# zhengchen1999/DOVE

Hardware: AMD Instinct MI355X
Metric: SR frames/s (33x720x1280 4x one-step, whole job) (higher is better)
Workload: dtype bf16; 1 GPU; synthetic 33x720x1280 HR clip (LR 180x320, 4x), one-step t=399, CogVideoX1.5-5B VAE + 42-layer DiT random-init, 1 clip per GPU (BASELINE configs[1]); weight_sums=True, vae_streams=2, variant=headline (bf16)

## Files before the change

### dove_amd/csrc/elementwise.hip

```cpp
#include "common.h"
#include "../../include/dove_hip.h"

__device__ __forceinline__ float load_any(const void* p, long long i, int dt) {
  return dt == DOVE_F32 ? ((const float*)p)[i] : bf2f(((const bf16_t*)p)[i]);
}
__device__ __forceinline__ void store_any(void* p, long long i, int dt, float v) {
  if (dt == DOVE_F32) ((float*)p)[i] = v;
  else ((bf16_t*)p)[i] = f2bf(v);
}

__global__ void cl_from_ncthw_kernel(const void* __restrict__ x, int dt, int C, long long npix, int Cp,
                                     float scale, float shift, bf16_t* __restrict__ y) {
  const long long p = (long long)blockIdx.x * blockDim.x + threadIdx.x;
  if (p >= npix) return;
  bf16_t* yr = y + p * Cp;
  for (int c0 = 0; c0 < Cp; c0 += 8) {
    float f[8];
#pragma unroll
    for (int e = 0; e < 8; ++e) {
      const int c = c0 + e;
      f[e] = c < C ? load_any(x, (long long)c * npix + p, dt) * scale + shift : 0.f;
    }
    *(uint4*)(yr + c0) = pack8(f);
  }
}

extern "C" int dove_cl_from_ncthw(const void* x, int dtype, int C, long long npix, int Cp, float scale, float shift,
                                   void* y, void* stream) {
  DOVE_CHECK_ARG(x && y, "cl_from_ncthw: null pointer");
  DOVE_CHECK_ARG(dtype == DOVE_F32 || dtype == DOVE_BF16, "cl_from_ncthw: bad dtype %d", dtype);
  DOVE_CHECK_ARG(Cp % 8 == 0 && Cp >= C && C > 0 && npix > 0, "cl_from_ncthw: need Cp %% 8 == 0, Cp >= C");
  hipLaunchKernelGGL(cl_from_ncthw_kernel, dim3((unsigned)((npix + 255) / 256)), dim3(256), 0, (hipStream_t)stream, x,
                     dtype, C, npix, Cp, scale, shift, (bf16_t*)y);
  DOVE_CHECK_LAUNCH("dove_cl_from_ncthw");
  return DOVE_OK;
}

__global__ void cl_im2col3x3_kernel(const void* __restrict__ x, int dt, int C, int T, int H, int W, int Cp, float scale, float shift,
                                    bf16_t* __restrict__ y) {
  const long long npix = (long long)T * H * W;
  const long long p = (long long)blockIdx.x * blockDim.x + threadIdx.x;
  if (p >= npix) return;
  const int w = (int)(p % W), h = (int)((p / W) % H);
  bf16_t* yr = y + p * Cp;
  for (int c0 = 0; c0 < Cp; c0 += 8) {
    float f[8];
#pragma unroll
    for (int e = 0; e < 8; ++e) {
      const int k = c0 + e, tap = k / C, c = k - tap * C;
      const int dy = tap / 3 - 1, dx = tap % 3 - 1;
      const bool in = tap < 9 && h + dy >= 0 && h + dy < H && w + dx >= 0 && w + dx < W;
      f[e] = in ? load_any(x, (long long)c * npix + p + (long long)dy * W + dx, dt) * scale + shift : 0.f;
    }
    *(uint4*)(yr + c0) = pack8(f);
  }
}
extern "C" int dove_cl_im2col3x3_from_ncthw(const void* x, int dtype, int C, int T, int H, int W, int Cp, float scale, float shift, void* y,
                                            void* stream) {
  DOVE_CHECK_ARG(x && y, "cl_im2col3x3: null pointer");
  DOVE_CHECK_ARG(dtype == DOVE_F32 || dtype == DOVE_BF16, "cl_im2col3x3: bad dtype %d", dtype);
  DOVE_CHECK_ARG(C > 0 && Cp % 8 == 0 && Cp >= 9 * C && T > 0 && H > 0 && W > 0, "cl_im2col3x3: need Cp %% 8 == 0 and Cp >= 9 C");
  const long long npix = (long long)T * H * W;
  hipLaunchKernelGGL(cl_im2col3x3_kernel, dim3((unsigned)((npix + 255) / 256)), dim3(256), 0, (hipStream_t)stream, x, dtype, C, T, H, W, Cp,
                     scale, shift, (bf16_t*)y);
  DOVE_CHECK_LAUNCH("dove_cl_im2col3x3_from_ncthw");
  return DOVE_OK;
}

__global__ void ncthw_from_cl_kernel(const bf16_t* __restrict__ x, long long ld, int C, long long npix, float scale,
                                     float shift, float lo, float hi, void* __restrict__ y, int dt) {
  const long long p = (long long)blockIdx.x * blockDim.x + threadIdx.x;
  if (p >= npix) return;
  const bf16_t* xr = x + p * ld;
  for (int c0 = 0; c0 < C; c0 += 4) {
    const uint2 v = *(const uint2*)(xr + c0);
    const float f[4] = {__uint_as_float(v.x << 16), __uint_as_float(v.x & 0xffff0000u), __uint_as_float(v.y << 16),
                        __uint_as_float(v.y & 0xffff0000u)};
#pragma unroll
    for (int e = 0; e < 4; ++e)
      if (c0 + e < C) store_any(y, (long long)(c0 + e) * npix + p, dt, fminf(fmaxf(f[e] * scale + shift, lo), hi));
  }
}

extern "C" int dove_ncthw_from_cl(const void* x, long long ld, int C, long long npix, float scale, float shift,
                                   float lo, float hi, void* y, int dtype, void* stream) {
  DOVE_CHECK_ARG(x && y, "ncthw_from_cl: null pointer");
  DOVE_CHECK_ARG(dtype == DOVE_F32 || dtype == DOVE_BF16, "ncthw_from_cl: bad dtype %d", dtype);
  DOVE_CHECK_ARG(ld % 4 == 0 && ld >= ((C + 3) / 4) * 4 && C > 0 && npix > 0, "ncthw_from_cl: ld must be a multiple of 4 covering C");
  hipLaunchKernelGGL(ncthw_from_cl_kernel, dim3((unsigned)((npix + 255) / 256)), dim3(256), 0, (hipStream_t)stream,
                     (const bf16_t*)x, ld, C, npix, scale, shift, lo, hi, y, dtype);
  DOVE_CHECK_LAUNCH("dove_ncthw_from_cl");
  return DOVE_OK;
}

__global__ __launch_bounds__(256) void conv_out_gather_kernel(const float* __restrict__ p, int ldp, int T, int H, int W, int C,
                                                              const float* __restrict__ bias, float scale, float shift, float lo, float hi,
                                                              void* __restrict__ y, int dt, int ldy) {
  extern __shared__ __attribute__((aligned(16))) float tile[];
  constexpr int TH = 8, TW = 64, RW = TW + 2, NREC = (TH + 2) * RW;
  const int lrec = ldp + 1, f4n = ldp >> 2;
  const int x0 = blockIdx.x * TW, y0 = blockIdx.y * TH, t = blockIdx.z;
  for (int i = threadIdx.x; i < NREC * f4n; i += 256) {
    const int rec = i / f4n, f4 = i - rec * f4n;
    const int ry = rec / RW, rx = rec - ry * RW;
    const int iy = y0 + ry - 1, ix = x0 + rx - 1;
    f32x4 v = {0.f, 0.f, 0.f, 0.f};
    if (iy >= 0 && iy < H && ix >= 0 && ix < W) v = *(const f32x4*)(p + (((long long)t * H + iy) * W + ix) * ldp + f4 * 4);
    float* d = tile + rec * lrec + f4 * 4;
    d[0] = v[0]; d[1] = v[1]; d[2] = v[2]; d[3] = v[3];
  }
  __syncthreads();
  const int lx = threadIdx.x & 63;
  const long long npix = (long long)T * H * W;
#pragma unroll
  for (int h2 = 0; h2 < 2; ++h2) {
    const int rr = (threadIdx.x >> 6) + 4 * h2;
    const int oy = y0 + rr, ox = x0 + lx;
    if (oy >= H || ox >= W) continue;
    float acc[4] = {0.f, 0.f, 0.f, 0.f};
#pragma unroll
    for (int dy = 0; dy < 3; ++dy)
#pragma unroll
      for (int dx = 0; dx < 3; ++dx) {
        const float* q = tile + ((rr + dy) * RW + lx + dx) * lrec + (dy * 3 + dx) * C;
        for (int c = 0; c < C; ++c) acc[c] += q[c];
      }
    const long long pix = ((long long)t * H + oy) * W + ox;
    if (ldy > 0) {
      bf16_t* yp = (bf16_t*)y + pix * ldy;
      for (int c = 0; c < ldy; ++c) yp[c] = c < C ? f2bf(acc[c] + (bias ? bias[c] : 0.f)) : (bf16_t)0;
      continue;
    }
    for (int c = 0; c < C; ++c) {
      const float v = bf2f(f2bf(acc[c] + (bias ? bias[c] : 0.f)));
      store_any(y, (long long)c * npix + pix, dt, fminf(fmaxf(v * scale + shift, lo), hi));
    }
  }
}
static int conv_out_gather_launch(const float* p, long long ldp, int T, int H, int W, int C, const float* bias, float scale, float shift,
                                  float lo, float hi, void* y, int dtype, int ldy, void* stream) {
  DOVE_CHECK_ARG(p && y, "conv_out_gather: null pointer");
  DOVE_CHECK_ARG(C >= 1 && C <= 4 && ldp >= 9 * C && ldp <= 36 && ldp % 4 == 0 && T > 0 && H > 0 && W > 0,
                 "conv_out_gather: need 1 <= C <= 4 and 9 C <= ldp <= 36, ldp %% 4 == 0");
  const int lds = 10 * 66 * ((int)ldp + 1) * 4;
  static PerDeviceOnce attr;
  if (auto once_ = attr.guard()) { (void)hipFuncSetAttribute((const void*)conv_out_gather_kernel, hipFuncAttributeMaxDynamicSharedMemorySize, 10 * 66 * 37 * 4); }
  dim3 grid((unsigned)((W + 63) / 64), (unsigned)((H + 7) / 8), (unsigned)T);
  hipLaunchKernelGGL(conv_out_gather_kernel, grid, dim3(256), lds, (hipStream_t)stream, p, (int)ldp, T, H, W, C, bias, scale, shift, lo, hi, y, dtype, ldy);
  DOVE_CHECK_LAUNCH("dove_conv_out_gather");
  return DOVE_OK;
}
extern "C" int dove_conv_out_gather(const float* p, long long ldp, int T, int H, int W, int C, const float* bias, float scale, float shift,
                                    float lo, float hi, void* y, int dtype, void* stream) {
  DOVE_CHECK_ARG(dtype == DOVE_F32 || dtype == DOVE_BF16, "conv_out_gather: bad dtype %d", dtype);
  return conv_out_gather_launch(p, ldp, T, H, W, C, bias, scale, shift, lo, hi, y, dtype, 0, stream);
}
extern "C" int dove_conv_out_gather_cl(const float* p, long long ldp, int T, int H, int W, int C, const float* bias, void* y, int ldy, void* stream) {
  DOVE_CHECK_ARG(ldy >= C && ldy <= 32 && ldy % 4 == 0, "conv_out_gather_cl: need C <= ldy <= 32, ldy %% 4 == 0 (got %d)", ldy);
  DOVE_CHECK_ARG(T <= 65535, "conv_out_gather_cl: more than 65535 frames (%d) in one call", T);
  return conv_out_gather_launch(p, ldp, T, H, W, C, bias, 1.0f, 0.0f, 0.0f, 0.0f, y, DOVE_BF16, ldy, stream);
}

__host__ __device__ inline int odd_to(int T) { return (T & 1) ? 1 + (T - 1) / 2 : T / 2; }
__global__ void avgpool_time_kernel(const bf16_t* __restrict__ x, int T, long long frame8, bf16_t* __restrict__ y) {
  const long long i = (long long)blockIdx.x * blockDim.x + threadIdx.x;
  if (i >= frame8) return;
  const int To = odd_to(T);
  const int inst = blockIdx.y / To, to = blockIdx.y - inst * To;
  const int odd = T & 1;
  const uint4* xs = (const uint4*)x + (long long)inst * T * frame8;
  uint4* ys = (uint4*)y + (long long)inst * To * frame8;
  if (odd && to == 0) {
    ys[i] = xs[i];
    return;
  }
  const int t0 = odd ? 1 + 2 * (to - 1) : 2 * to;
  float a[8], b[8];
  unpack8(xs[(long long)t0 * frame8 + i], a);
  unpack8(xs[(long long)(t0 + 1) * frame8 + i], b);
#pragma unroll
  for (int e = 0; e < 8; ++e) a[e] = 0.5f * (a[e] + b[e]);
  ys[(long long)to * frame8 + i] = pack8(a);
}

extern "C" int dove_avgpool_time_nb_bf16(const void* x, int nb, int T, long long frame_elems, void* y, void* stream) {
  DOVE_CHECK_ARG(x && y, "avgpool_time: null pointer");
  DOVE_CHECK_ARG(T >= 2 && frame_elems % 8 == 0 && frame_elems > 0, "avgpool_time: need T >= 2 and frame_elems %% 8 == 0");
  const int To = odd_to(T);
  DOVE_CHECK_ARG(nb >= 1 && (long long)nb * To <= 65535, "avgpool_time: bad instance count %d", nb);
  const long long f8 = frame_elems / 8;
  hipLaunchKernelGGL(avgpool_time_kernel, dim3((unsigned)((f8 + 255) / 256), nb * To), dim3(256), 0, (hipStream_t)stream,
                     (const bf16_t*)x, T, f8, (bf16_t*)y);
  DOVE_CHECK_LAUNCH("dove_avgpool_time_bf16");
  return DOVE_OK;
}
extern "C" int dove_avgpool_time_bf16(const void* x, int T, long long frame_elems, void* y, void* stream) {
  return dove_avgpool_time_nb_bf16(x, 1, T, frame_elems, y, stream);
}

__global__ void posterior_kernel(const bf16_t* __restrict__ mom, long long ld, int L, long long npix,
                                 const void* __restrict__ noise, int ndt, void* __restrict__ out, int odt) {
  const long long p = (long long)blockIdx.x * blockDim.x + threadIdx.x;
  if (p >= npix) return;
  for (int c = 0; c < L; ++c) {
    const float mean = bf2f(mom[p * ld + c]);
    float lv = bf2f(mom[p * ld + L + c]);
    lv = fminf(fmaxf(lv, -30.f), 20.f);
    const float eps = load_any(noise, (long long)c * npix + p, ndt);
    store_any(out, (long long)c * npix + p, odt, mean + __expf(0.5f * lv) * eps);
  }
}

extern "C" int dove_posterior_sample(const void* moments, long long ld, int latent_channels, long long npix,
                                      const void* noise, int noise_dtype, void* out, int out_dtype, void* stream) {
  DOVE_CHECK_ARG(moments && noise && out, "posterior_sample: null pointer");
  DOVE_CHECK_ARG(ld >= 2 * latent_channels && npix > 0, "posterior_sample: bad ld");
  hipLaunchKernelGGL(posterior_kernel, dim3((unsigned)((npix + 255) / 256)), dim3(256), 0, (hipStream_t)stream,
                     (const bf16_t*)moments, ld, latent_channels, npix, noise, noise_dtype, out, out_dtype);
  DOVE_CHECK_LAUNCH("dove_posterior_sample");
  return DOVE_OK;
}

__global__ void axpby_kernel(const void* x, const void* y, void* out, int dt, long long n, float a, float b) {
  const long long i = (long long)blockIdx.x * blockDim.x + threadIdx.x;
  if (i >= n) return;
  store_any(out, i, dt, a * load_any(x, i, dt) + b * load_any(y, i, dt));
}

extern "C" int dove_axpby(const void* x, const void* y, void* out, int dtype, long long n, float a, float b,
                           void* stream) {
  DOVE_CHECK_ARG(x && y && out && n > 0, "axpby: null pointer / empty");
  DOVE_CHECK_ARG(dtype == DOVE_F32 || dtype == DOVE_BF16, "axpby: bad dtype %d", dtype);
  hipLaunchKernelGGL(axpby_kernel, dim3((unsigned)((n + 255) / 256)), dim3(256), 0, (hipStream_t)stream, x, y, out,
                     dtype, n, a, b);
  DOVE_CHECK_LAUNCH("dove_axpby");
  return DOVE_OK;
}

__global__ void patchify_kernel(const void* __restrict__ x, int dt, int T, int C, int H, int W, int pt, int p,
                                bf16_t* __restrict__ tok, long long ld, int dir, void* __restrict__ y) {
  const int gh = H / p, gw = W / p;
  const int F = C * pt * p * p;
  const long long total = (long long)(T / pt) * gh * gw * F;
  const long long i = (long long)blockIdx.x * blockDim.x + threadIdx.x;
  if (i >= total) return;
  const int f = (int)(i % F);
  const long long n = i / F;
  const int pw = f % p, ph = (f / p) % p, tt = (f / (p * p)) % pt, c = f / (p * p * pt);
  const int iw = (int)(n % gw), ih = (int)((n / gw) % gh), it = (int)(n / ((long long)gw * gh));
  const long long src = (((long long)(it * pt + tt) * C + c) * H + ih * p + ph) * W + iw * p + pw;
  if (dir == 0) tok[n * ld + f] = f2bf(load_any(x, src, dt));
  else store_any(y, src, dt, bf2f(tok[n * ld + f]));
}

extern "C" int dove_patchify(const void* x, int dtype, int T, int C, int H, int W, int pt, int p, void* tokens,
                              long long ld, void* stream) {
  DOVE_CHECK_ARG(x && tokens, "patchify: null pointer");
  DOVE_CHECK_ARG(T % pt == 0 && H % p == 0 && W % p == 0 && ld >= (long long)C * pt * p * p, "patchify: shape not divisible by patch");
  const long long total = (long long)(T / pt) * (H / p) * (W / p) * C * pt * p * p;
  hipLaunchKernelGGL(patchify_kernel, dim3((unsigned)((total + 255) / 256)), dim3(256), 0, (hipStream_t)stream, x,
                     dtype, T, C, H, W, pt, p, (bf16_t*)tokens, ld, 0, nullptr);
  DOVE_CHECK_LAUNCH("dove_patchify");
  return DOVE_OK;
}

extern "C" int dove_unpatchify(const void* tokens, long long ld, int T, int C, int H, int W, int pt, int p, void* y,
                                int dtype, void* stream) {
  DOVE_CHECK_ARG(y && tokens, "unpatchify: null pointer");
  DOVE_CHECK_ARG(T % pt == 0 && H % p == 0 && W % p == 0 && ld >= (long long)C * pt * p * p, "unpatchify: shape not divisible by patch");
  const long long total = (long long)(T / pt) * (H / p) * (W / p) * C * pt * p * p;
  hipLaunchKernelGGL(patchify_kernel, dim3((unsigned)((total + 255) / 256)), dim3(256), 0, (hipStream_t)stream,
                     nullptr, dtype, T, C, H, W, pt, p, (bf16_t*)const_cast<void*>(tokens), ld, 1, y);
  DOVE_CHECK_LAUNCH("dove_unpatchify");
  return DOVE_OK;
}

__global__ __launch_bounds__(256) void gemv_kernel(const bf16_t* __restrict__ W, const float* __restrict__ b,
                                                   const float* __restrict__ x, int in_f, int out_f, int act,
                                                   float* __restrict__ y) {
  const int lane = threadIdx.x & 63;
  const int j = blockIdx.x * 4 + (threadIdx.x >> 6);
  if (j >= out_f) return;
  const bf16_t* wr = W + (long long)j * in_f;
  float acc = 0.f;
  for (int k0 = lane * 8; k0 < in_f; k0 += 512) {
    float w[8];
    unpack8(*(const uint4*)(wr + k0), w);
#pragma unroll
    for (int e = 0; e < 8; ++e) {
      float xv = x[k0 + e];
      if (act == 1) xv = silu_f(xv);
      acc += w[e] * xv;
    }
  }
  acc = wave_sum(acc);
  if (lane == 0) y[j] = acc + (b ? b[j] : 0.f);
}

extern "C" int dove_gemv_bf16(const void* W, const float* bias, const float* x, int in_features, int out_features,
                               int act_in, float* y, void* stream) {
  DOVE_CHECK_ARG(W && x && y, "gemv: null pointer");
// ... 169 lines not shown
```

### dove_amd/csrc/norm.hip

```cpp
#include "common.h"
#include "../../include/dove_hip.h"

__global__ __launch_bounds__(256) void gn_partial_kernel(const bf16_t* __restrict__ xall, long long npix, int C,
                                                         int cpp_log, float* __restrict__ partial_all) {
  const bf16_t* __restrict__ x = xall + (long long)blockIdx.y * npix * C;
  float* __restrict__ partial = partial_all + (long long)blockIdx.y * gridDim.x * 64;
  __shared__ float red[256 * 17];
  __shared__ float chan[2 * 2048];
  const int tid = threadIdx.x;
  const int cpp = 1 << cpp_log;
  const int q = tid & (cpp - 1), sub = tid >> cpp_log;
  const int nsub = 256 >> cpp_log;
  float s[8], ss[8];
#pragma unroll
  for (int e = 0; e < 8; ++e) { s[e] = 0.f; ss[e] = 0.f; }
  for (long long p = (long long)blockIdx.x * nsub + sub; p < npix; p += (long long)gridDim.x * nsub) {
    const uint4 v = *(const uint4*)(x + p * C + q * 8);
    float f[8];
    unpack8(v, f);
#pragma unroll
    for (int e = 0; e < 8; ++e) { s[e] += f[e]; ss[e] += f[e] * f[e]; }
  }
  float* r = red + (q * nsub + sub) * 17;
#pragma unroll
// ... 130 lines not shown
  while ((1 << cpp_log) < C / 8) ++cpp_log;
  const int nsub = 256 >> cpp_log;
  long long bpf = (frame_pix + (long long)nsub * 32 - 1) / ((long long)nsub * 32);
  if (bpf > 256) bpf = 256;
  if (bpf * frames > ws_blocks) {
    dove_set_error("%s: %lld frames x %lld blocks per frame exceed the %d scratch rows", who, frames, bpf, ws_blocks);
    return 0;
  }
  hipLaunchKernelGGL(gn_partial_kernel, dim3((unsigned)bpf, (unsigned)frames), dim3(256), 0, s, (const bf16_t*)x, frame_pix, C, cpp_log,
                     (float*)partial_ws);
  return (int)(bpf * frames);
}

extern "C" int dove_groupnorm_stats_bf16(const void* x, long long npix, long long frame_pix, int C, float eps, void* partial_ws,
                                          int ws_blocks, float* stats, void* stream) {
  DOVE_CHECK_ARG(x && partial_ws && stats, "groupnorm_stats: null pointer");
  hipStream_t s = (hipStream_t)stream;
  const int rows = gn_partial_launch(x, npix, frame_pix, C, partial_ws, ws_blocks, s, "groupnorm_stats");
  if (!rows) return DOVE_EINVAL;
  DOVE_CHECK_LAUNCH("dove_groupnorm_stats_bf16(partial)");
  hipLaunchKernelGGL(gn_finalize_kernel<float>, dim3(1), dim3(256), 0, s, (const float*)partial_ws, rows,
                     (double)npix * (double)(C / 32), eps, stats);
  DOVE_CHECK_LAUNCH("dove_groupnorm_stats_bf16(finalize)");
  return DOVE_OK;
}

extern "C" int dove_groupnorm_stats_nb_bf16(const void* x, int nb, long long npix, long long frame_pix, int C, float eps, void* partial_ws,
                                             int ws_blocks, float* stats, void* stream) {
  DOVE_CHECK_ARG(x && partial_ws && stats && nb >= 1, "groupnorm_stats: null pointer");
  hipStream_t s = (hipStream_t)stream;
  const int rows = gn_partial_launch(x, npix * nb, frame_pix > 0 ? frame_pix : npix, C, partial_ws, ws_blocks, s, "groupnorm_stats");
  if (!rows) return DOVE_EINVAL;
  DOVE_CHECK_LAUNCH("dove_groupnorm_stats_bf16(partial)");
  DOVE_CHECK_ARG(rows % nb == 0, "groupnorm_stats: %d partial rows do not split over %d instances", rows, nb);
  hipLaunchKernelGGL(gn_finalize_kernel<float>, dim3(nb), dim3(256), 0, s, (const float*)partial_ws, rows / nb,
                     (double)npix * (double)(C / 32), eps, stats);
  DOVE_CHECK_LAUNCH("dove_groupnorm_stats_bf16(finalize)");
  return DOVE_OK;
}

extern "C" int dove_groupnorm_sums_bf16(const void* x, long long npix, long long frame_pix, int C, void* partial_ws, int ws_blocks,
                                        double* sums, void* stream) {
  DOVE_CHECK_ARG(x && partial_ws && sums, "groupnorm_sums: null pointer");
  hipStream_t s = (hipStream_t)stream;
  const int rows = gn_partial_launch(x, npix, frame_pix, C, partial_ws, ws_blocks, s, "groupnorm_sums");
  if (!rows) return DOVE_EINVAL;
  DOVE_CHECK_LAUNCH("dove_groupnorm_sums_bf16(partial)");
  hipLaunchKernelGGL(gn_sums_kernel<float>, dim3(1), dim3(256), 0, s, (const float*)partial_ws, rows, sums);
  DOVE_CHECK_LAUNCH("dove_groupnorm_sums_bf16(sums)");
  return DOVE_OK;
}

struct GnApplyArgs {
  const bf16_t* x; bf16_t* y; const float* stats; const float* gamma; const float* beta;
  const bf16_t* yb;
  int T, H, W, C, cpp_log;
  int hz, wz, sshift;
  int tmap[32];
  int act;
  int Tz;
};

__global__ __launch_bounds__(256) void gn_apply_kernel(const GnApplyArgs a) {
  const int tid = threadIdx.x;
  const int cpp = 1 << a.cpp_log;
  const int q = tid & (cpp - 1), sub = tid >> a.cpp_log;
  const int nsub = 256 >> a.cpp_log;
  const int cpg = a.C / 32;
  const int t = blockIdx.y;
  const int b = t / a.T;
  const float* __restrict__ stats = a.stats + b * 64;
  float sc[8], sh[8];
#pragma unroll
  for (int e = 0; e < 8; ++e) {
    const int ch = q * 8 + e, g = ch / cpg;
    const float mean = stats[g * 2], rstd = stats[g * 2 + 1];
    sc[e] = rstd * a.gamma[ch];
    sh[e] = a.beta[ch] - mean * sc[e];
  }
  const int tz = b * a.Tz + a.tmap[t - b * a.T];
  for (int h = blockIdx.x; h < a.H; h += gridDim.x) {
    const long long rowbase = ((long long)t * a.H + h) * a.W;
    const long long zrow = ((long long)tz * a.hz + (h >> a.sshift)) * a.wz;
    for (int w0 = sub; w0 < a.W; w0 += 4 * nsub) {
      uint4 xv[4], yv[4], bv[4];
#pragma unroll
      for (int u = 0; u < 4; ++u) {
        const int w = w0 + u * nsub;
        if (w < a.W) {
          xv[u] = *(const uint4*)(a.x + (rowbase + w) * a.C + q * 8);
          if (a.yb) {
            const bf16_t* yb = a.yb + (zrow + (w >> a.sshift)) * (2 * a.C) + q * 8;
            yv[u] = *(const uint4*)yb;
            bv[u] = *(const uint4*)(yb + a.C);
          }
        }
      }
#pragma unroll
      for (int u = 0; u < 4; ++u) {
        const int w = w0 + u * nsub;
        if (w < a.W) {
          float f[8];
          unpack8(xv[u], f);
#pragma unroll
          for (int e = 0; e < 8; ++e) f[e] = f[e] * sc[e] + sh[e];
          if (a.yb) {
            float fy[8], fb[8];
            unpack8(yv[u], fy);
            unpack8(bv[u], fb);
#pragma unroll
            for (int e = 0; e < 8; ++e) f[e] = f[e] * fy[e] + fb[e];
          }
          if (a.act) {
#pragma unroll
            for (int e = 0; e < 8; ++e) f[e] = silu_f(f[e]);
          }
          *(uint4*)(a.y + (rowbase + w) * a.C + q * 8) = pack8(f);
        }
      }
    }
  }
}

extern "C" int dove_groupnorm_apply_nb_bf16(const void* x, void* y, int nb, int T, int H, int W, int C, const float* stats,
                                             const float* gamma, const float* beta, int silu, const void* yb, int Tz, int hz,
                                             int wz, int sshift, const int* tmap, void* stream) {
  DOVE_CHECK_ARG(x && y && stats && gamma && beta, "groupnorm_apply: null pointer");
  DOVE_CHECK_ARG(nb >= 1 && (long long)nb * T <= 65535, "groupnorm_apply: bad instance count %d", nb);
  DOVE_CHECK_ARG(C >= 32 && C <= 2048 && (C & (C - 1)) == 0, "groupnorm_apply: C (%d) must be a power of two in [32,2048]", C);
  DOVE_CHECK_ARG(T > 0 && T <= 32 && H > 0 && W > 0, "groupnorm_apply: need 0 < T <= 32 frames per batch (got %d), H, W > 0", T);
  GnApplyArgs a;
  a.x = (const bf16_t*)x; a.y = (bf16_t*)y; a.stats = stats; a.gamma = gamma; a.beta = beta; a.yb = (const bf16_t*)yb;
  a.T = T; a.H = H; a.W = W; a.C = C; a.act = silu;
  int cpp_log = 0;
  while ((1 << cpp_log) < C / 8) ++cpp_log;
  a.cpp_log = cpp_log;
  a.hz = hz; a.wz = wz; a.sshift = sshift; a.Tz = Tz;
  for (int i = 0; i < 32; ++i) a.tmap[i] = 0;
  if (yb) {
    DOVE_CHECK_ARG(tmap, "groupnorm_apply: spatial norm needs a frame map");
    DOVE_CHECK_ARG(sshift >= 0 && sshift <= 8 && (hz << sshift) >= H && (wz << sshift) >= W, "groupnorm_apply: latent grid too small");
    for (int i = 0; i < T; ++i) a.tmap[i] = tmap[i];
  }
  hipLaunchKernelGGL(gn_apply_kernel, dim3(H < 4096 ? H : 4096, nb * T), dim3(256), 0, (hipStream_t)stream, a);
  DOVE_CHECK_LAUNCH("dove_groupnorm_apply_bf16");
  return DOVE_OK;
}
extern "C" int dove_groupnorm_apply_bf16(const void* x, void* y, int T, int H, int W, int C, const float* stats,
                                          const float* gamma, const float* beta, int silu, const void* yb, int hz,
                                          int wz, int sshift, const int* tmap, void* stream) {
  return dove_groupnorm_apply_nb_bf16(x, y, 1, T, H, W, C, stats, gamma, beta, silu, yb, 0, hz, wz, sshift, tmap, stream);
}

template <int NIT>
__global__ __launch_bounds__(256) void ln_mod_kernel(const bf16_t* __restrict__ x, bf16_t* __restrict__ y,
                                                     long long rows, int D, float eps,
                                                     const float* __restrict__ gamma, const float* __restrict__ beta,
                                                     const float* __restrict__ mod, long long split) {
  extern __shared__ __attribute__((aligned(16))) float lnp[];
  float* A = lnp;
  float* Bv = lnp + 2 * D;
  for (int c = threadIdx.x; c < D; c += 256) {
    const float g = gamma[c], b = beta[c];
#pragma unroll
    for (int cls = 0; cls < 2; ++cls) {
      float sc = 0.f, sh = 0.f;
      if (mod) { sh = mod[(long long)cls * 2 * D + c]; sc = mod[(long long)cls * 2 * D + D + c]; }
      A[cls * D + c] = g * (1.0f + sc);
      Bv[cls * D + c] = b * (1.0f + sc) + sh;
    }
  }
  __syncthreads();
  const int lane = threadIdx.x & 63, wave = threadIdx.x >> 6;
  for (int r = 0; r < 8; ++r) {
    const long long row = (long long)blockIdx.x * 32 + wave * 8 + r;
    if (row >= rows) break;
    const bf16_t* xr = x + row * D;
    float f[NIT][8];
    float s = 0.f;
#pragma unroll
    for (int i = 0; i < NIT; ++i) {
      const int c0 = (i * 64 + lane) * 8;
      if (c0 < D) {
        unpack8(*(const uint4*)(xr + c0), f[i]);
#pragma unroll
        for (int e = 0; e < 8; ++e) s += f[i][e];
      } else {
#pragma unroll
        for (int e = 0; e < 8; ++e) f[i][e] = 0.f;
      }
    }
    const float mean = wave_sum(s) / (float)D;
    float v = 0.f;
#pragma unroll
    for (int i = 0; i < NIT; ++i) {
      const int c0 = (i * 64 + lane) * 8;
      if (c0 < D) {
#pragma unroll
        for (int e = 0; e < 8; ++e) { const float d = f[i][e] - mean; v += d * d; }
      }
    }
    const float rstd = rsqrtf(wave_sum(v) / (float)D + eps);
    const int cls = row < split ? 0 : 1;
    bf16_t* yr = y + row * D;
#pragma unroll
    for (int i = 0; i < NIT; ++i) {
      const int c0 = (i * 64 + lane) * 8;
      if (c0 < D) {
        const f32x4 a0 = *(const f32x4*)(A + cls * D + c0), a1 = *(const f32x4*)(A + cls * D + c0 + 4);
        const f32x4 b0 = *(const f32x4*)(Bv + cls * D + c0), b1 = *(const f32x4*)(Bv + cls * D + c0 + 4);
        float o[8];
#pragma unroll
        for (int e = 0; e < 4; ++e) {
          o[e] = (f[i][e] - mean) * rstd * a0[e] + b0[e];
          o[4 + e] = (f[i][4 + e] - mean) * rstd * a1[e] + b1[e];
        }
        *(uint4*)(yr + c0) = pack8(o);
      }
    }
  }
}

extern "C" int dove_layernorm_modulate_bf16(const void* x, void* y, long long rows, int D, float eps,
                                             const float* gamma, const float* beta, const float* mod,
                                             long long split, void* stream) {
  DOVE_CHECK_ARG(x && y && gamma && beta, "layernorm_modulate: null pointer");
  DOVE_CHECK_ARG(D % 8 == 0 && D > 0 && D <= 4096, "layernorm_modulate: D (%d) must be a multiple of 8, <= 4096", D);
  DOVE_CHECK_ARG(rows > 0, "layernorm_modulate: empty input");
  const int nit = (D + 511) / 512;
  const unsigned grid = (unsigned)((rows + 31) / 32);
  const size_t lds = (size_t)4 * D * sizeof(float);
  hipStream_t s = (hipStream_t)stream;
#define LN_LAUNCH(N)                                                                                          \
  hipLaunchKernelGGL((ln_mod_kernel<N>), dim3(grid), dim3(256), lds, s, (const bf16_t*)x, (bf16_t*)y, rows, D, eps, \
                     gamma, beta, mod, split)
  switch (nit) {
    case 1: LN_LAUNCH(1); break;
    case 2: LN_LAUNCH(2); break;
    case 3: LN_LAUNCH(3); break;
    case 4: LN_LAUNCH(4); break;
    case 5: LN_LAUNCH(5); break;
    case 6: LN_LAUNCH(6); break;
    case 7: LN_LAUNCH(7); break;
    default: LN_LAUNCH(8); break;
  }
#undef LN_LAUNCH
  DOVE_CHECK_LAUNCH("dove_layernorm_modulate_bf16");
  return DOVE_OK;
}

constexpr int QK_HB = 8;
__global__ __launch_bounds__(256) void qk_post_kernel(const bf16_t* __restrict__ qkv, long long N, long long Npad, int heads, int text_len,
                                                      const float* __restrict__ gq, const float* __restrict__ bq,
                                                      const float* __restrict__ gk, const float* __restrict__ bk,
                                                      const float* __restrict__ cosT, const float* __restrict__ sinT, float qscale, float eps,
                                                      bf16_t* __restrict__ Qh, bf16_t* __restrict__ Kh, float* __restrict__ norm2) {
  __shared__ unsigned smax[4][QK_HB];
  const int c = threadIdx.x & 7;
  const int h0 = blockIdx.y * QK_HB, which = blockIdx.z;
  const long long n = (long long)blockIdx.x * 32 + (threadIdx.x >> 3);
  const int D = heads * 64;
  const bool live = n < N;
  const long long nn = live ? n : N - 1;
  const float* gam = (which == 0 ? gq : gk) + c * 8;
  const float* bet = (which == 0 ? bq : bk) + c * 8;
  const f32x4 g0 = *(const f32x4*)gam, g1 = *(const f32x4*)(gam + 4), b0 = *(const f32x4*)bet, b1 = *(const f32x4*)(bet + 4);
  const bool rope = nn >= text_len && cosT;
  f32x4 c0 = {1.f, 1.f, 1.f, 1.f}, c1 = c0, s0 = {0.f, 0.f, 0.f, 0.f}, s1 = s0;
  if (rope) {
    const float* cr = cosT + (nn - text_len) * 64 + c * 8;
    const float* sr = sinT + (nn - text_len) * 64 + c * 8;
    c0 = *(const f32x4*)cr; c1 = *(const f32x4*)(cr + 4); s0 = *(const f32x4*)sr; s1 = *(const f32x4*)(sr + 4);
  }
  const float sc = which == 0 ? qscale : 1.0f;
  const bf16_t* src = qkv + nn * (3LL * D) + (long long)which * D + c * 8;
  bf16_t* dst = (which == 0 ? Qh : Kh) + nn * 64 + c * 8;
  uint4 raw[QK_HB];
#pragma unroll
  for (int j = 0; j < QK_HB; ++j) raw[j] = h0 + j < heads ? *(const uint4*)(src + (h0 + j) * 64) : uint4{0u, 0u, 0u, 0u};
#pragma unroll
  for (int j = 0; j < QK_HB; ++j) {
    float f[8];
    unpack8(raw[j], f);
    float s = 0.f;
#pragma unroll
    for (int e = 0; e < 8; ++e) s += f[e];
    s += __shfl_xor(s, 1); s += __shfl_xor(s, 2); s += __shfl_xor(s, 4);
    const float mean = s * (1.0f / 64.0f);
    float v = 0.f;
#pragma unroll
    for (int e = 0; e < 8; ++e) { const float t = f[e] - mean; v += t * t; }
    v += __shfl_xor(v, 1); v += __shfl_xor(v, 2); v += __shfl_xor(v, 4);
    const float rstd = rsqrtf(v * (1.0f / 64.0f) + eps);
#pragma unroll
    for (int e = 0; e < 8; ++e) f[e] = (f[e] - mean) * rstd * (e < 4 ? g0[e] : g1[e - 4]) + (e < 4 ? b0[e] : b1[e - 4]);
    if (rope) {
#pragma unroll
      for (int i = 0; i < 4; ++i) {
        const float a = f[2 * i], b = f[2 * i + 1];
        const float ca = i < 2 ? c0[2 * i] : c1[2 * i - 4], cb = i < 2 ? c0[2 * i + 1] : c1[2 * i - 3];
        const float sa = i < 2 ? s0[2 * i] : s1[2 * i - 4], sb = i < 2 ? s0[2 * i + 1] : s1[2 * i - 3];
        f[2 * i] = a * ca - b * sa;
        f[2 * i + 1] = b * cb + a * sb;
      }
    }
#pragma unroll
    for (int e = 0; e < 8; ++e) f[e] *= sc;
    const uint4 packed = pack8(f);
    if (live && h0 + j < heads) *(uint4*)(dst + (long long)(h0 + j) * Npad * 64) = packed;
    if (norm2) {
      float r[8];
      unpack8(packed, r);
      float q = 0.f;
#pragma unroll
      for (int e = 0; e < 8; ++e) q += r[e] * r[e];
      q += __shfl_xor(q, 1); q += __shfl_xor(q, 2); q += __shfl_xor(q, 4);
      unsigned qb = __float_as_uint(q);
      qb = max(qb, (unsigned)__shfl_xor((int)qb, 8)); qb = max(qb, (unsigned)__shfl_xor((int)qb, 16)); qb = max(qb, (unsigned)__shfl_xor((int)qb, 32));
      if ((threadIdx.x & 63) == 0) smax[threadIdx.x >> 6][j] = qb;
    }
  }
  if (norm2) {
    __syncthreads();
    const int j = threadIdx.x;
    if (j < QK_HB && h0 + j < heads) {
      atomicMax((unsigned*)(norm2 + (h0 + j) * 2 + which), max(max(smax[0][j], smax[1][j]), max(smax[2][j], smax[3][j])));
    }
  }
}

__global__ __launch_bounds__(256) void v_post_kernel(const bf16_t* __restrict__ qkv, long long N, long long Npad, int heads,
                                                     bf16_t* __restrict__ Vt, int v_swap) {
  __shared__ float vt[4][64][65];
  const int lane = threadIdx.x & 63, wave = threadIdx.x >> 6;
  const int h = blockIdx.y;
  const long long n0 = ((long long)blockIdx.x * 4 + wave) * 64;
  if (n0 >= N) return;
  const int D = heads * 64;
  const int t8 = lane >> 3, c = lane & 7;
#pragma unroll
  for (int i = 0; i < 8; ++i) {
    const long long n = n0 + i * 8 + t8;
    float f[8];
    if (n < N) unpack8(*(const uint4*)(qkv + n * (3LL * D) + 2LL * D + h * 64 + c * 8), f);
    else {
#pragma unroll
      for (int e = 0; e < 8; ++e) f[e] = 0.f;
    }
#pragma unroll
    for (int e = 0; e < 8; ++e) vt[wave][i * 8 + t8][c * 8 + e] = f[e];
  }
  __builtin_amdgcn_wave_barrier();
  asm volatile("s_waitcnt lgkmcnt(0)" ::: "memory");
  if ((Npad & 7) == 0) {
    bf16_t* dst = Vt + ((long long)h * 64 + lane) * Npad + n0;
#pragma unroll
    for (int j = 0; j < 8; ++j) {
      float o[8];
      const int g16 = (j >> 1) * 16, odd = (j & 1) * 4;
#pragma unroll
      for (int e = 0; e < 8; ++e) o[e] = v_swap ? vt[wave][g16 + odd + (e & 3) + (e >> 2) * 8][lane] : vt[wave][j * 8 + e][lane];
      if (n0 + j * 8 + 8 <= Npad) *(uint4*)(dst + j * 8) = pack8(o);
    }
  } else {
    bf16_t* dst = Vt + ((long long)h * 64 + lane) * Npad + n0;
    for (int j = 0; j < 64 && n0 + j < N; ++j) dst[j] = f2bf(vt[wave][j][lane]);
  }
}

extern "C" int dove_qkv_post_bf16(const void* qkv, long long N, long long Npad, int heads, int head_dim, int text_len,
                                   const float* gq, const float* bq, const float* gk, const float* bk,
                                   const float* cosT, const float* sinT, float qscale, float eps, void* Qh, void* Kh,
                                   void* Vt, int v_order, float* norm2, void* stream) {
  DOVE_CHECK_ARG(qkv && Qh && Kh && Vt && gq && bq && gk && bk, "qkv_post: null pointer");
  DOVE_CHECK_ARG(head_dim == 64, "qkv_post: head_dim must be 64 (got %d)", head_dim);
  DOVE_CHECK_ARG(N > 0 && Npad >= N, "qkv_post: Npad must be >= N");
  DOVE_CHECK_ARG((cosT == nullptr) == (sinT == nullptr), "qkv_post: cos/sin must both be given or both be null");
  DOVE_CHECK_ARG(v_order == 0 || (v_order == 1 && Npad % 16 == 0), "qkv_post: v_order 1 (quad-swapped V^T) needs Npad %% 16 == 0");
  if (norm2) {
    const hipError_t me = hipMemsetAsync(norm2, 0, sizeof(float) * 2 * heads, (hipStream_t)stream);
    if (me != hipSuccess) { dove_set_error("qkv_post: clearing norm2 failed: %s", hipGetErrorString(me)); return DOVE_ELAUNCH; }
  }
  hipLaunchKernelGGL(qk_post_kernel, dim3((unsigned)((N + 31) / 32), (unsigned)((heads + QK_HB - 1) / QK_HB), 2), dim3(256), 0, (hipStream_t)stream, (const bf16_t*)qkv, N, Npad, heads,
                     text_len, gq, bq, gk, bk, cosT, sinT, qscale, eps, (bf16_t*)Qh, (bf16_t*)Kh, norm2);
  hipLaunchKernelGGL(v_post_kernel, dim3((unsigned)((N + 255) / 256), heads), dim3(256), 0, (hipStream_t)stream, (const bf16_t*)qkv, N, Npad, heads,
                     (bf16_t*)Vt, v_order);
  DOVE_CHECK_LAUNCH("dove_qkv_post_bf16");
  return DOVE_OK;
}

__global__ __launch_bounds__(256) void vt_quad_swap_kernel(uint4* __restrict__ vt, long long ngroups) {
  const long long g = (long long)blockIdx.x * 256 + threadIdx.x;
  if (g >= ngroups) return;
  const uint4 a = vt[2 * g], b = vt[2 * g + 1];
  vt[2 * g] = uint4{a.x, a.y, b.x, b.y};
  vt[2 * g + 1] = uint4{a.z, a.w, b.z, b.w};
}
extern "C" int dove_vt_quad_swap_bf16(void* Vt, long long rows, long long Npad, void* stream) {
  DOVE_CHECK_ARG(Vt && rows > 0 && Npad > 0 && Npad % 16 == 0, "vt_quad_swap: Npad must be a positive multiple of 16");
  const long long ng = rows * (Npad / 16);
  hipLaunchKernelGGL(vt_quad_swap_kernel, dim3((unsigned)((ng + 255) / 256)), dim3(256), 0, (hipStream_t)stream, (uint4*)Vt, ng);
  DOVE_CHECK_LAUNCH("dove_vt_quad_swap_bf16");
  return DOVE_OK;
}

struct UlyPlaceArgs {
  const bf16_t *rq, *rk, *rv;
  bf16_t *Qh, *Kh, *Vt;
  int world, hloc;
  long long N, Npad;
  long long bound[17];
  long long off[17];
  int extra;
  float* norm2_out;
};
__device__ __forceinline__ int uly_rank(const UlyPlaceArgs& a, long long n) {
  int i = 0;
  while (i + 1 < a.world && n >= a.bound[i + 1]) ++i;
  return i;
}
__global__ __launch_bounds__(256) void ulysses_place_kernel(const UlyPlaceArgs a) {
  const long long t = (long long)blockIdx.x * 256 + threadIdx.x;
  if (blockIdx.y == 3) {
    if (t >= a.hloc * 2) return;
    const int h = (int)(t >> 1), e = (int)(t & 1);
    unsigned m = 0u;
    for (int i = 0; i < a.world; ++i) {
      const long long ci = a.bound[i + 1] - a.bound[i];
      m = max(m, ((const unsigned*)(a.rk + a.off[i] + ((long long)h * (ci + 1) + ci) * 64))[e]);
    }
    ((unsigned*)a.norm2_out)[t] = m;
    return;
  }
  if (blockIdx.y < 2) {
    const long long total = (long long)a.hloc * a.N * 8;
    if (t >= total) return;
    const int c = (int)(t & 7);
    const long long n = (t >> 3) % a.N;
    const int h = (int)((t >> 3) / a.N);
    const int i = uly_rank(a, n);
    const long long ci = a.bound[i + 1] - a.bound[i] + a.extra;
    const bf16_t* src = (blockIdx.y == 0 ? a.rq : a.rk) + a.off[i] + ((long long)h * ci + (n - a.bound[i])) * 64 + c * 8;
    bf16_t* dst = (blockIdx.y == 0 ? a.Qh : a.Kh) + ((long long)h * a.Npad + n) * 64 + c * 8;
    *(uint4*)dst = *(const uint4*)src;
  } else {
    const long long quads = a.Npad >> 2, total = (long long)a.hloc * 64 * quads;
    if (t >= total) return;
    const long long qd = t % quads;
    const long long row = t / quads;
    const int h = (int)(row >> 6), d = (int)(row & 63);
    bf16_t v[4];
#pragma unroll
    for (int e = 0; e < 4; ++e) {
      const long long n = qd * 4 + e;
      v[e] = 0;
      if (n < a.N) {
        const int i = uly_rank(a, n);
        const long long ci = a.bound[i + 1] - a.bound[i] + a.extra;
        v[e] = a.rv[a.off[i] + ((long long)h * 64 + d) * ci + (n - a.bound[i])];
      }
    }
    const int q = (int)(qd & 3);
    const long long pq = (qd & ~3ll) | (q == 1 ? 2 : (q == 2 ? 1 : q));
    uint2 w;
    w.x = (uint32_t)v[0] | ((uint32_t)v[1] << 16);
    w.y = (uint32_t)v[2] | ((uint32_t)v[3] << 16);
    *(uint2*)(a.Vt + row * a.Npad + pq * 4) = w;
  }
}
extern "C" int dove_ulysses_place_bf16(const void* rq, const void* rk, const void* rv, const long long* counts, int world, int hloc, long long N,
                                       long long Npad, void* Qh, void* Kh, void* Vt, float* norm2_out, void* stream) {
  DOVE_CHECK_ARG(rq && rk && rv && counts && Qh && Kh && Vt, "ulysses_place: null pointer");
  DOVE_CHECK_ARG(world >= 1 && world <= 16 && hloc >= 1 && N > 0 && Npad >= N && Npad % 16 == 0, "ulysses_place: bad shape (world %d, hloc %d)", world, hloc);
  UlyPlaceArgs a;
  a.rq = (const bf16_t*)rq; a.rk = (const bf16_t*)rk; a.rv = (const bf16_t*)rv;
  a.Qh = (bf16_t*)Qh; a.Kh = (bf16_t*)Kh; a.Vt = (bf16_t*)Vt;
  a.world = world; a.hloc = hloc; a.N = N; a.Npad = Npad;
  long long b = 0, o = 0;
  for (int i = 0; i < 17; ++i) { a.bound[i] = N; a.off[i] = 0; }
  for (int i = 0; i < world; ++i) {
    DOVE_CHECK_ARG(counts[i] >= 0, "ulysses_place: negative row count");
    a.bound[i] = b; a.off[i] = o;
    b += counts[i]; o += (counts[i] + (norm2_out ? 1 : 0)) * hloc * 64;
  }
  a.extra = norm2_out ? 1 : 0;
  a.norm2_out = norm2_out;
  a.bound[world] = b;
  DOVE_CHECK_ARG(b == N, "ulysses_place: the ranks' row counts add up to %lld, not N = %lld", b, N);
  const long long tq = (long long)hloc * N * 8, tv = (long long)hloc * 64 * (Npad >> 2);
  const long long tmax = tq > tv ? tq : tv;
  dim3 grid((unsigned)((tmax + 255) / 256), norm2_out ? 4 : 3);
  hipLaunchKernelGGL(ulysses_place_kernel, grid, dim3(256), 0, (hipStream_t)stream, a);
  DOVE_CHECK_LAUNCH("dove_ulysses_place_bf16");
  return DOVE_OK;
}
```

Measured before the change: 34.90 frames/s.

## Tile im2col/conv-out gather through LDS, prefetch LN rows, coalesce V^T stores

Adds a shared-memory strip kernel for the 3-channel im2col so that each input pixel is read once per tile instead of nine times. Templates the conv-out gather on C, dropping the padded LDS stride and issuing loads ahead of the LDS writes. The layernorm-modulate kernel now processes 16-row blocks of a single class, halving its LDS tables and prefetching the next row into registers. The V-transpose writes are remapped so that lanes store contiguous 16-byte chunks along N rather than striding by Npad per lane. These are several unrelated memory-access changes to small kernels, and they add templated code paths whose edge cases (split clamping, unaligned Npad) carry some correctness risk.

```diff
diff --git a/dove_amd/csrc/elementwise.hip b/dove_amd/csrc/elementwise.hip
--- a/dove_amd/csrc/elementwise.hip
+++ b/dove_amd/csrc/elementwise.hip
@@ -55,14 +55,63 @@
     *(uint4*)(yr + c0) = pack8(f);
   }
 }
+constexpr int IM_TW = 64, IM_TH = 4;
+template <int C, int CP>
+__global__ __launch_bounds__(256) void cl_im2col3x3_strip_kernel(const void* __restrict__ x, int dt, int T, int H, int W, float scale, float shift,
+                                                                 bf16_t* __restrict__ y) {
+  constexpr int RW = IM_TW + 2, RH = IM_TH + 2, NP = CP / 8;
+  static_assert(CP % 8 == 0 && CP >= 9 * C && 256 / NP == IM_TW && 256 % NP == 0, "one pass of the workgroup = one row of the strip");
+  __shared__ float tile[C * RH * RW];
+  const int x0 = blockIdx.x * IM_TW, y0 = blockIdx.y * IM_TH, t = blockIdx.z;
+  const long long npix = (long long)T * H * W;
+  constexpr int NIT = (C * RH * RW + 255) / 256;
+  float v[NIT];
+#pragma unroll
+  for (int it = 0; it < NIT; ++it) {
+    const int i = it * 256 + threadIdx.x;
+    const int c = i / (RH * RW), rem = i - c * (RH * RW), ry = rem / RW, rx = rem - ry * RW;
+    const int iy = y0 + ry - 1, ix = x0 + rx - 1;
+    const bool in = i < C * RH * RW && iy >= 0 && iy < H && ix >= 0 && ix < W;
+    v[it] = in ? load_any(x, (long long)c * npix + ((long long)t * H + iy) * W + ix, dt) * scale + shift : 0.f;
+  }
+#pragma unroll
+  for (int it = 0; it < NIT; ++it) {
+    const int i = it * 256 + threadIdx.x;
+    if (i < C * RH * RW) tile[i] = v[it];
+  }
+  __syncthreads();
+  const int piece = threadIdx.x % NP, px = threadIdx.x / NP;
+  int off[8];
+#pragma unroll
+  for (int e = 0; e < 8; ++e) {
+    const int k = piece * 8 + e, tap = k / C, c = k - tap * C, dy = tap / 3, dx = tap - dy * 3;
+    off[e] = tap < 9 ? (c * RH + dy) * RW + dx : -1;
+  }
+  const int ox = x0 + px;
+  if (ox >= W) return;
+#pragma unroll
+  for (int ry = 0; ry < IM_TH; ++ry) {
+    const int oy = y0 + ry;
+    if (oy >= H) break;
+    float f[8];
+#pragma unroll
+    for (int e = 0; e < 8; ++e) f[e] = off[e] >= 0 ? tile[off[e] + ry * RW + px] : 0.f;
+    *(uint4*)(y + (((long long)t * H + oy) * W + ox) * CP + piece * 8) = pack8(f);
+  }
+}
 extern "C" int dove_cl_im2col3x3_from_ncthw(const void* x, int dtype, int C, int T, int H, int W, int Cp, float scale, float shift, void* y,
                                             void* stream) {
   DOVE_CHECK_ARG(x && y, "cl_im2col3x3: null pointer");
   DOVE_CHECK_ARG(dtype == DOVE_F32 || dtype == DOVE_BF16, "cl_im2col3x3: bad dtype %d", dtype);
   DOVE_CHECK_ARG(C > 0 && Cp % 8 == 0 && Cp >= 9 * C && T > 0 && H > 0 && W > 0, "cl_im2col3x3: need Cp %% 8 == 0 and Cp >= 9 C");
   const long long npix = (long long)T * H * W;
-  hipLaunchKernelGGL(cl_im2col3x3_kernel, dim3((unsigned)((npix + 255) / 256)), dim3(256), 0, (hipStream_t)stream, x, dtype, C, T, H, W, Cp,
-                     scale, shift, (bf16_t*)y);
+  if (C == 3 && Cp == 32 && T <= 65535 && (H + IM_TH - 1) / IM_TH <= 65535) {
+    hipLaunchKernelGGL((cl_im2col3x3_strip_kernel<3, 32>), dim3((unsigned)((W + IM_TW - 1) / IM_TW), (unsigned)((H + IM_TH - 1) / IM_TH), (unsigned)T),
+                       dim3(256), 0, (hipStream_t)stream, x, dtype, T, H, W, scale, shift, (bf16_t*)y);
+  } else {
+    hipLaunchKernelGGL(cl_im2col3x3_kernel, dim3((unsigned)((npix + 255) / 256)), dim3(256), 0, (hipStream_t)stream, x, dtype, C, T, H, W, Cp,
+                       scale, shift, (bf16_t*)y);
+  }
   DOVE_CHECK_LAUNCH("dove_cl_im2col3x3_from_ncthw");
   return DOVE_OK;
 }
@@ -93,21 +142,28 @@
   return DOVE_OK;
 }
 
-__global__ __launch_bounds__(256) void conv_out_gather_kernel(const float* __restrict__ p, int ldp, int T, int H, int W, int C,
+template <int C>
+__global__ __launch_bounds__(256) void conv_out_gather_kernel(const float* __restrict__ p, int ldp, int T, int H, int W,
                                                               const float* __restrict__ bias, float scale, float shift, float lo, float hi,
                                                               void* __restrict__ y, int dt, int ldy) {
   extern __shared__ __attribute__((aligned(16))) float tile[];
-  constexpr int TH = 8, TW = 64, RW = TW + 2, NREC = (TH + 2) * RW;
-  const int lrec = ldp + 1, f4n = ldp >> 2;
+  constexpr int TH = 8, TW = 64, RW = TW + 2, NREC = (TH + 2) * RW, NS = (9 * C + 3) / 4, NIT = (NREC * NS + 255) / 256;
+  f32x4* tile4 = (f32x4*)tile;
   const int x0 = blockIdx.x * TW, y0 = blockIdx.y * TH, t = blockIdx.z;
-  for (int i = threadIdx.x; i < NREC * f4n; i += 256) {
-    const int rec = i / f4n, f4 = i - rec * f4n;
+  f32x4 v[NIT];
+#pragma unroll
+  for (int it = 0; it < NIT; ++it) {
+    const int i = it * 256 + threadIdx.x;
+    const int rec = i / NS, f4 = i - rec * NS;
     const int ry = rec / RW, rx = rec - ry * RW;
     const int iy = y0 + ry - 1, ix = x0 + rx - 1;
-    f32x4 v = {0.f, 0.f, 0.f, 0.f};
-    if (iy >= 0 && iy < H && ix >= 0 && ix < W) v = *(const f32x4*)(p + (((long long)t * H + iy) * W + ix) * ldp + f4 * 4);
-    float* d = tile + rec * lrec + f4 * 4;
-    d[0] = v[0]; d[1] = v[1]; d[2] = v[2]; d[3] = v[3];
+    v[it] = f32x4{0.f, 0.f, 0.f, 0.f};
+    if (i < NREC * NS && iy >= 0 && iy < H && ix >= 0 && ix < W) v[it] = *(const f32x4*)(p + (((long long)t * H + iy) * W + ix) * ldp + f4 * 4);
+  }
+#pragma unroll
+  for (int it = 0; it < NIT; ++it) {
+    const int i = it * 256 + threadIdx.x;
+    if (i < NREC * NS) tile4[i] = v[it];
   }
   __syncthreads();
   const int lx = threadIdx.x & 63;
@@ -117,36 +173,55 @@
     const int rr = (threadIdx.x >> 6) + 4 * h2;
     const int oy = y0 + rr, ox = x0 + lx;
     if (oy >= H || ox >= W) continue;
-    float acc[4] = {0.f, 0.f, 0.f, 0.f};
+    float acc[C];
+#pragma unroll
+    for (int c = 0; c < C; ++c) acc[c] = 0.f;
 #pragma unroll
     for (int dy = 0; dy < 3; ++dy)
 #pragma unroll
       for (int dx = 0; dx < 3; ++dx) {
-        const float* q = tile + ((rr + dy) * RW + lx + dx) * lrec + (dy * 3 + dx) * C;
-        for (int c = 0; c < C; ++c) acc[c] += q[c];
+        const int k0 = (dy * 3 + dx) * C;
+        const f32x4* q = tile4 + ((rr + dy) * RW + lx + dx) * NS;
+        const f32x4 qa = q[k0 >> 2], qb = q[(k0 + C - 1) >> 2];
+#pragma unroll
+        for (int c = 0; c < C; ++c) acc[c] += ((k0 + c) >> 2) == (k0 >> 2) ? qa[(k0 + c) & 3] : qb[(k0 + c) & 3];
       }
     const long long pix = ((long long)t * H + oy) * W + ox;
     if (ldy > 0) {
       bf16_t* yp = (bf16_t*)y + pix * ldy;
-      for (int c = 0; c < ldy; ++c) yp[c] = c < C ? f2bf(acc[c] + (bias ? bias[c] : 0.f)) : (bf16_t)0;
+#pragma unroll
+      for (int c = 0; c < C; ++c) yp[c] = f2bf(acc[c] + (bias ? bias[c] : 0.f));
+      for (int c = C; c < ldy; ++c) yp[c] = (bf16_t)0;
       continue;
     }
+#pragma unroll
     for (int c = 0; c < C; ++c) {
-      const float v = bf2f(f2bf(acc[c] + (bias ? bias[c] : 0.f)));
-      store_any(y, (long long)c * npix + pix, dt, fminf(fmaxf(v * scale + shift, lo), hi));
+      const float o = bf2f(f2bf(acc[c] + (bias ? bias[c] : 0.f)));
+      store_any(y, (long long)c * npix + pix, dt, fminf(fmaxf(o * scale + shift, lo), hi));
     }
   }
+}
+template <int C>
+static void conv_out_gather_launch_c(dim3 grid, hipStream_t stream, const float* p, int ldp, int T, int H, int W, const float* bias, float scale,
+                                     float shift, float lo, float hi, void* y, int dtype, int ldy) {
+  constexpr int lds = 10 * 66 * ((9 * C + 3) / 4) * 16;
+  static PerDeviceOnce attr;
+  if (auto once_ = attr.guard()) { (void)hipFuncSetAttribute((const void*)conv_out_gather_kernel<C>, hipFuncAttributeMaxDynamicSharedMemorySize, lds); }
+  hipLaunchKernelGGL((conv_out_gather_kernel<C>), grid, dim3(256), lds, stream, p, ldp, T, H, W, bias, scale, shift, lo, hi, y, dtype, ldy);
 }
 static int conv_out_gather_launch(const float* p, long long ldp, int T, int H, int W, int C, const float* bias, float scale, float shift,
                                   float lo, float hi, void* y, int dtype, int ldy, void* stream) {
   DOVE_CHECK_ARG(p && y, "conv_out_gather: null pointer");
   DOVE_CHECK_ARG(C >= 1 && C <= 4 && ldp >= 9 * C && ldp <= 36 && ldp % 4 == 0 && T > 0 && H > 0 && W > 0,
                  "conv_out_gather: need 1 <= C <= 4 and 9 C <= ldp <= 36, ldp %% 4 == 0");
-  const int lds = 10 * 66 * ((int)ldp + 1) * 4;
-  static PerDeviceOnce attr;
-  if (auto once_ = attr.guard()) { (void)hipFuncSetAttribute((const void*)conv_out_gather_kernel, hipFuncAttributeMaxDynamicSharedMemorySize, 10 * 66 * 37 * 4); }
   dim3 grid((unsigned)((W + 63) / 64), (unsigned)((H + 7) / 8), (unsigned)T);
-  hipLaunchKernelGGL(conv_out_gather_kernel, grid, dim3(256), lds, (hipStream_t)stream, p, (int)ldp, T, H, W, C, bias, scale, shift, lo, hi, y, dtype, ldy);
+  hipStream_t s = (hipStream_t)stream;
+  switch (C) {
+    case 1: conv_out_gather_launch_c<1>(grid, s, p, (int)ldp, T, H, W, bias, scale, shift, lo, hi, y, dtype, ldy); break;
+    case 2: conv_out_gather_launch_c<2>(grid, s, p, (int)ldp, T, H, W, bias, scale, shift, lo, hi, y, dtype, ldy); break;
+    case 3: conv_out_gather_launch_c<3>(grid, s, p, (int)ldp, T, H, W, bias, scale, shift, lo, hi, y, dtype, ldy); break;
+    default: conv_out_gather_launch_c<4>(grid, s, p, (int)ldp, T, H, W, bias, scale, shift, lo, hi, y, dtype, ldy); break;
+  }
   DOVE_CHECK_LAUNCH("dove_conv_out_gather");
   return DOVE_OK;
 }
diff --git a/dove_amd/csrc/norm.hip b/dove_amd/csrc/norm.hip
--- a/dove_amd/csrc/norm.hip
+++ b/dove_amd/csrc/norm.hip
@@ -306,6 +306,7 @@
   return dove_groupnorm_apply_nb_bf16(x, y, 1, T, H, W, C, stats, gamma, beta, silu, yb, 0, hz, wz, sshift, tmap, stream);
 }
 
+constexpr int LN_ROWS = 16;
 template <int NIT>
 __global__ __launch_bounds__(256) void ln_mod_kernel(const bf16_t* __restrict__ x, bf16_t* __restrict__ y,
                                                      long long rows, int D, float eps,
@@ -313,35 +314,59 @@
                                                      const float* __restrict__ mod, long long split) {
   extern __shared__ __attribute__((aligned(16))) float lnp[];
   float* A = lnp;
-  float* Bv = lnp + 2 * D;
-  for (int c = threadIdx.x; c < D; c += 256) {
-    const float g = gamma[c], b = beta[c];
-#pragma unroll
-    for (int cls = 0; cls < 2; ++cls) {
-      float sc = 0.f, sh = 0.f;
-      if (mod) { sh = mod[(long long)cls * 2 * D + c]; sc = mod[(long long)cls * 2 * D + D + c]; }
-      A[cls * D + c] = g * (1.0f + sc);
-      Bv[cls * D + c] = b * (1.0f + sc) + sh;
-    }
+  float* Bv = lnp + D;
+  const int lane = threadIdx.x & 63, wave = threadIdx.x >> 6;
+  const long long nb0 = (split + LN_ROWS - 1) / LN_ROWS;
+  const int cls = blockIdx.x < nb0 ? 0 : 1;
+  const long long first = cls == 0 ? (long long)blockIdx.x * LN_ROWS : split + ((long long)blockIdx.x - nb0) * LN_ROWS;
+  const long long end = cls == 0 ? split : rows;
+  constexpr int RW = LN_ROWS / 4;
+  const long long row0 = first + wave * RW;
+  uint4 raw[NIT];
+  if (row0 < end) {
+#pragma unroll
+    for (int i = 0; i < NIT; ++i) {
+      const int c0 = (i * 64 + lane) * 8;
+      if (c0 < D) raw[i] = *(const uint4*)(x + row0 * D + c0);
+    }
+  }
+  for (int c = threadIdx.x * 4; c < D; c += 1024) {
+    const f32x4 g4 = *(const f32x4*)(gamma + c), b4 = *(const f32x4*)(beta + c);
+    f32x4 sh4 = {0.f, 0.f, 0.f, 0.f}, sc4 = sh4;
+    if (mod) { sh4 = *(const f32x4*)(mod + (long long)cls * 2 * D + c); sc4 = *(const f32x4*)(mod + (long long)cls * 2 * D + D + c); }
+    f32x4 a4, o4;
+#pragma unroll
+    for (int e = 0; e < 4; ++e) {
+      const float g = g4[e], b = b4[e], sc = sc4[e], sh = sh4[e];
+      a4[e] = g * (1.0f + sc);
+      o4[e] = b * (1.0f + sc) + sh;
+    }
+    *(f32x4*)(A + c) = a4;
+    *(f32x4*)(Bv + c) = o4;
   }
   __syncthreads();
-  const int lane = threadIdx.x & 63, wave = threadIdx.x >> 6;
-  for (int r = 0; r < 8; ++r) {
-    const long long row = (long long)blockIdx.x * 32 + wave * 8 + r;
-    if (row >= rows) break;
-    const bf16_t* xr = x + row * D;
+  for (int r = 0; r < RW; ++r) {
+    const long long row = row0 + r;
+    if (row >= end) break;
     float f[NIT][8];
     float s = 0.f;
 #pragma unroll
     for (int i = 0; i < NIT; ++i) {
       const int c0 = (i * 64 + lane) * 8;
       if (c0 < D) {
-        unpack8(*(const uint4*)(xr + c0), f[i]);
+        unpack8(raw[i], f[i]);
 #pragma unroll
         for (int e = 0; e < 8; ++e) s += f[i][e];
       } else {
 #pragma unroll
         for (int e = 0; e < 8; ++e) f[i][e] = 0.f;
+      }
+    }
+    if (r + 1 < RW && row + 1 < end) {
+#pragma unroll
+      for (int i = 0; i < NIT; ++i) {
+        const int c0 = (i * 64 + lane) * 8;
+        if (c0 < D) raw[i] = *(const uint4*)(x + (row + 1) * D + c0);
       }
     }
     const float mean = wave_sum(s) / (float)D;
@@ -355,14 +380,13 @@
       }
     }
     const float rstd = rsqrtf(wave_sum(v) / (float)D + eps);
-    const int cls = row < split ? 0 : 1;
     bf16_t* yr = y + row * D;
 #pragma unroll
     for (int i = 0; i < NIT; ++i) {
       const int c0 = (i * 64 + lane) * 8;
       if (c0 < D) {
-        const f32x4 a0 = *(const f32x4*)(A + cls * D + c0), a1 = *(const f32x4*)(A + cls * D + c0 + 4);
-        const f32x4 b0 = *(const f32x4*)(Bv + cls * D + c0), b1 = *(const f32x4*)(Bv + cls * D + c0 + 4);
+        const f32x4 a0 = *(const f32x4*)(A + c0), a1 = *(const f32x4*)(A + c0 + 4);
+        const f32x4 b0 = *(const f32x4*)(Bv + c0), b1 = *(const f32x4*)(Bv + c0 + 4);
         float o[8];
 #pragma unroll
         for (int e = 0; e < 4; ++e) {
@@ -382,8 +406,9 @@
   DOVE_CHECK_ARG(D % 8 == 0 && D > 0 && D <= 4096, "layernorm_modulate: D (%d) must be a multiple of 8, <= 4096", D);
   DOVE_CHECK_ARG(rows > 0, "layernorm_modulate: empty input");
   const int nit = (D + 511) / 512;
-  const unsigned grid = (unsigned)((rows + 31) / 32);
-  const size_t lds = (size_t)4 * D * sizeof(float);
+  split = !mod || split < 0 ? 0 : split > rows ? rows : split;
+  const unsigned grid = (unsigned)((split + LN_ROWS - 1) / LN_ROWS + (rows - split + LN_ROWS - 1) / LN_ROWS);
+  const size_t lds = (size_t)2 * D * sizeof(float);
   hipStream_t s = (hipStream_t)stream;
 #define LN_LAUNCH(N)                                                                                          \
   hipLaunchKernelGGL((ln_mod_kernel<N>), dim3(grid), dim3(256), lds, s, (const bf16_t*)x, (bf16_t*)y, rows, D, eps, \
@@ -507,18 +532,22 @@
   __builtin_amdgcn_wave_barrier();
   asm volatile("s_waitcnt lgkmcnt(0)" ::: "memory");
   if ((Npad & 7) == 0) {
-    bf16_t* dst = Vt + ((long long)h * 64 + lane) * Npad + n0;
-#pragma unroll
-    for (int j = 0; j < 8; ++j) {
+    const int g16 = (c >> 1) * 16, odd = (c & 1) * 4;
+    const bool inside = n0 + c * 8 + 8 <= Npad;
+    bf16_t* dst = Vt + ((long long)h * 64 + t8) * Npad + n0 + c * 8;
+#pragma unroll
+    for (int i = 0; i < 8; ++i) {
       float o[8];
-      const int g16 = (j >> 1) * 16, odd = (j & 1) * 4;
-#pragma unroll
-      for (int e = 0; e < 8; ++e) o[e] = v_swap ? vt[wave][g16 + odd + (e & 3) + (e >> 2) * 8][lane] : vt[wave][j * 8 + e][lane];
-      if (n0 + j * 8 + 8 <= Npad) *(uint4*)(dst + j * 8) = pack8(o);
+#pragma unroll
+      for (int e = 0; e < 8; ++e) o[e] = v_swap ? vt[wave][g16 + odd + (e & 3) + (e >> 2) * 8][i * 8 + t8] : vt[wave][c * 8 + e][i * 8 + t8];
+      if (inside) *(uint4*)(dst + (long long)i * 8 * Npad) = pack8(o);
     }
   } else {
-    bf16_t* dst = Vt + ((long long)h * 64 + lane) * Npad + n0;
-    for (int j = 0; j < 64 && n0 + j < N; ++j) dst[j] = f2bf(vt[wave][j][lane]);
+    if (n0 + lane < N) {
+      bf16_t* dst = Vt + (long long)h * 64 * Npad + n0 + lane;
+#pragma unroll 8
+      for (int d = 0; d < 64; ++d) dst[(long long)d * Npad] = f2bf(vt[wave][lane][d]);
+    }
   }
 }
 
```

Result: no change. 35.10 frames/s (median of 6 runs) (+0.6%).
